# haoyu94/RoITr

Measured on AMD Instinct MI355X. Metric: point-cloud pairs/s, higher is better.
Workload: dtype f32; 1 GPU; 3DMatch-sized synthetic pairs: 5000 pts/cloud src+tgt, fp32, 3DMatch test settings (P=256 patches x 64 pts, 100 Sinkhorn iterations), full RIGA_v2 forward; n_points=5000, weights=closed-form, variant 'selective' (roitr_amd/weights.py); normals: field, cloud=uniform, correspondences_found=66241517

## Files before the change

### include/roitr_engine.h

```cpp
#ifndef ROITR_ENGINE_H
#define ROITR_ENGINE_H

#include <stddef.h>

#ifdef __cplusplus
extern "C" {
#endif

#ifndef ROITR_POINTOPS_H
typedef struct ihipStream_t* roitr_stream_t;
#endif

typedef struct RoitrGemm {
    int M, N, K;
    const float* A; const float* A2; int lda; const int* a_idx; int a_limit;
    const float* W; int ldw; const int* w_idx; int w_limit;
    const float* bias; float alpha; int relu;
    float* C; int ldc;
    int batch; long sA, sW, sC, sBias, sAidx, sWidx;
    const int* seg_off; int seg_a0, seg_w0;
    const float* ln_gamma; const float* ln_beta; const float* ln_res; const int* ln_res_idx; const float* ln_post;
    int ln_relu; float ln_eps;
    int bf16;
    const float* A_cat; int lda_cat; int k_cat;
// ... 24 lines not shown
                      roitr_stream_t stream);
int roitr_segment_mean(int b, int C, const float* x, const int* offset, float* out, roitr_stream_t stream);
int roitr_sinusoid(long rows, int C, const float* vals, const float* div_term, float* out, roitr_stream_t stream);
int roitr_geo_embed(long rows, int C, int angle_k, const float* d_idx, const float* a_idx, const float* div_term,
                    const float* Wd, const float* bd, const float* Wa, const float* ba, float* out, roitr_stream_t stream);
int roitr_split3_bf16(long n, const float* src, unsigned short* dst, roitr_stream_t stream);
int roitr_geo_embed_split(long rows, int C, int angle_k, const float* d_idx, const float* a_idx, const float* div_term,
                          const unsigned short* Wd3, const float* bd, const unsigned short* Wa3, const float* ba, float* out,
                          roitr_stream_t stream);
int roitr_geo_embed_bf16(long rows, int C, int angle_k, const float* d_idx, const float* a_idx, const float* div_term,
                         const unsigned short* Wd, const float* bd, const unsigned short* Wa, const float* ba, float* out,
                         roitr_stream_t stream);
int roitr_geo_embed_bf16_out(long rows, int C, int angle_k, const float* d_idx, const float* a_idx, const float* div_term,
                             const unsigned short* Wd, const float* bd, const unsigned short* Wa, const float* ba,
                             unsigned short* out, roitr_stream_t stream);
size_t roitr_geo_table_floats(int C, int n_int_d, int n_int_a);
int roitr_geo_table_build(int C, const float* div_term, const float* Wd, const float* bd, const float* Wa, const float* ba,
                          float interval, int n_int_d, int n_int_a, float* table, double* fit);
int roitr_geo_embed_table(long rows, int C, int angle_k, const float* d_idx, const float* a_idx, const float* table, float interval,
                          int n_int_d, int n_int_a, const float* div_term, const float* Wd, const float* bd, const float* Wa,
                          const float* ba, void* out, int out_bf16, roitr_stream_t stream);
int roitr_geo_combine(long rows, int C, int k, const float* pd, const float* pa, float* out, roitr_stream_t stream);
int roitr_gather_rows(long rows, int C, const float* in, const int* idx, int limit, float* out, roitr_stream_t stream);
int roitr_compose_idx(int n, const int* outer, const int* inner, int* out, roitr_stream_t stream);
int roitr_calc_ppf(int m, int k, const float* centre_xyz, const float* centre_normals, const float* ref_xyz,
                   const float* ref_normals, const int* group_idx, float* out, roitr_stream_t stream);

typedef struct RoitrLocalAttn {
    int M, K, H, heads;
    const float* q; int ldq;
    const float* k; int ldk;
    const float* v; int ldv;
    const int* group_idx; const float* ppf;
    const float* wvpe; const float* bvpe;
    float scale;
    float* out; int ldo;
    const void* node_order;
    int bf16;
    const float* wpe; const float* bpe;
} RoitrLocalAttn;
int roitr_local_attention(const RoitrLocalAttn* a, roitr_stream_t stream);
int roitr_build_pfold(int H, int heads, const float* wpe, const float* bpe, float* pfold, roitr_stream_t stream);

typedef struct RoitrLocalAttnFold {
    int M, in_dim, H;
    const float* x; int ldx;
// ... 59 lines not shown
int roitr_local_weights_reorder_host(const float* src, int rows, int k, int ldw, float* dst);

int roitr_geo_indices(int rows, const float* pts, const int* offset, const int* cloud_of_row, const long* eoff,
                      float sigma_d, float sigma_a, int angle_k, int n_max, float* d_idx, float* a_idx, roitr_stream_t stream);

typedef struct RoitrMha {
    int q_row0, q_rows, C, heads;
    const float* q; int ldq;
    const float* k; int ldk;
    const float* v; int ldv;
    const int* offset; const int* cloud_of_row; const int* partner;
    const float* E; const long* eoff; const float* qt; const float* bp;
    float scale; int nk_max;
    float* out; int ldo;
    float* ebar;
    int e_bf16;
} RoitrMha;
int roitr_mha(const RoitrMha* a, roitr_stream_t stream);


int roitr_point_to_node_partition(int b, int n_points, int n_nodes, const float* pts, const int* pt_offset,
                                  const float* nodes, const int* node_offset, const int* cloud_of_node, int limit,
                                  int* p2n, float* p2n_dist, int* node_masks, int* knn_idx, int* knn_mask, roitr_stream_t stream);

typedef struct RoitrCoarse {
    int pairs, C, num_corr, dual_norm, max_ref, max_src;
    const float* feats; const int* node_offset; const int* node_masks;
    float* scratch; long scratch_stride;
    int* tgt_corr; int* src_corr; float* corr_scores; int* n_corr;
    const float* xy; long xy_stride; int xy_ld;
    int lds_cap;
} RoitrCoarse;
size_t roitr_coarse_scratch_floats(int n_ref, int n_src);
int roitr_coarse_matching(const RoitrCoarse* a, roitr_stream_t stream);
int roitr_adaptive_matching(const RoitrCoarse* a, int min_num, float threshold, roitr_stream_t stream);

int roitr_patch_offsets(int pairs, const int* n_corr, int slots, int* pair_off, roitr_stream_t stream);

typedef struct RoitrPatch {
    int pairs, num_corr, limit;
    const int* n_corr; const int* tgt_corr; const int* src_corr;
    const int* node_offset; const int* pt_offset; const int* knn_idx; const int* knn_mask; const float* points;
    int* tgt_rows; int* src_rows; int* tgt_masks; int* src_masks; float* tgt_pts; float* src_pts;
    const int* pair_off; int slots;
} RoitrPatch;
int roitr_patch_gather(const RoitrPatch* a, roitr_stream_t stream);
// ... 73 lines not shown
    float* matching_scores;
    float* out_tgt_pts; float* out_src_pts; float* out_scores; int* out_patch;
    int* fine_offsets;
    int* n_out;
    float* gt_node_occ;
    int* gt_corr_idx;
    float* gt_corr_overlaps;
    int* gt_corr_count;
    void* inputs_ready;
    int* patch_offsets;
    int* pair_starts;
    int patch_slots;
} RoitrForwardIO;

void* roitr_engine_create(const RoitrEngineConfig* cfg);
void roitr_engine_destroy(void* engine);
int roitr_engine_set_param(void* engine, const char* name, const float* device_ptr, long numel);
int roitr_engine_finalize(void* engine, roitr_stream_t stream);
int roitr_engine_geo_table_info(void* engine, double* info);
int roitr_engine_forward(void* engine, const RoitrForwardIO* io, roitr_stream_t stream);
int roitr_engine_forward_graph(void* engine, const RoitrForwardIO* io, roitr_stream_t stream);
int roitr_engine_graph_count(void* engine);
int roitr_engine_set_phase_overlap(void* engine, int on);
int roitr_engine_scratch_info(void* engine, long* out5);
int roitr_engine_set_tap(void* engine, const char* name, void* device_ptr);
int roitr_engine_set_inject(void* engine, const char* name, const void* device_ptr);
void roitr_level_sizes(int n, int* out4);


int roitr_inlier_counts(int pairs, const int* starts, const float* src_pts, const float* tgt_pts, const float* rot,
                        const float* trans, float radius, int* inliers, roitr_stream_t stream);
int roitr_coarse_hits(int pairs, int num_corr, const int* n_corr, const int* tgt_corr, const int* src_corr, int gt_cap,
                      const int* gt_idx, const float* gt_overlaps, const int* gt_count, float acceptance_overlap, int* hits,
                      roitr_stream_t stream);


size_t roitr_registration_workspace_bytes(int pairs, int total_rows, int iterations, int chunks);
int roitr_ransac_correspondences(int pairs, const int* starts, int total_rows, const float* src_pts, const float* tgt_pts,
                                 const float* scores, const unsigned int* pair_keys, int sample_mode, int n_points, int ransac_n,
                                 float distance_threshold, float edge_similarity, int iterations, int refine_iters, int refine_weighted,
                                 unsigned long long seed, int chunks, void* workspace, size_t workspace_bytes, float* transforms,
                                 int* inliers, int* best_iteration, int* valid_hypotheses, int* n_used, int* selected,
                                 roitr_stream_t stream);
int roitr_ransac_samples(int pairs, const int* n, const unsigned int* pair_keys, unsigned long long seed, int it0, int count, int* out,
                         roitr_stream_t stream);
int roitr_weighted_procrustes(int batch, int n, const float* src_pts, const float* tgt_pts, const float* weights, float weight_thresh,
// ... 57 lines not shown
```

### roitr_amd/csrc/engine.cpp

```cpp
#include <hip/hip_runtime.h>
#include <math.h>
#include <stdio.h>
#include <string.h>

#include <map>
#include <string>
#include <vector>

#include "common.h"
#include "prof.h"
#include "roitr_engine.h"
#include "roitr_pointops.h"

#define CHK(x)                    \
    do {                          \
        int s__ = (x);            \
        if (s__ != 0) return s__; \
    } while (0)

namespace {

constexpr int HEADS = 4;
constexpr int GRID_MIN_POINTS = 768;

// ... 87 lines not shown
    hipStream_t side = nullptr;
    enum Ev {
        EV_MAIN_BEGIN,
        EV_LEVEL2_GEOM_DONE,
        EV_LEVEL3_GEOM_DONE,
        EV_LEVEL4_GEOM_DONE,
        EV_LEVEL1_WS_FREE,
        EV_EMBED_DONE,
        EV_NN3_DONE,
        EV_TAIL_DONE,
        EV_ERROR_JOIN,
        EV_DESC_COPIED,
        EV_LEVEL1_GROUPS_READY,
        EV_ENCODER_DONE,
        EV_BRANCH_DONE,
        EV_BRANCH_ERROR_JOIN,
        NEV
    };
    static Ev ev_level_done(int l) { return (Ev)(EV_LEVEL2_GEOM_DONE + l - 1); }
    hipEvent_t ev[NEV] = {};
    bool side_forked = false;
    hipStream_t branch = nullptr;
    int phase_overlap = 1;
    bool branch_forked = false;
    bool on_branch = false;
    std::string err;
    hipStream_t fin_stream = nullptr;
    struct GraphEntry {
        std::vector<long> key;
        hipGraph_t graph = nullptr; hipGraphExec_t exec = nullptr;
        char* pin = nullptr; size_t pin_cap = 0;
        long epoch = -1;
        bool warmed = false, failed = false;
        unsigned long stamp = 0;
    };
    std::vector<GraphEntry> graphs;
    long arena_epoch = 0;
    unsigned long graph_clock = 0;
    char* capture_pin = nullptr;
    std::map<std::pair<const float*, long>, unsigned short*> x3;
    std::vector<const float*> frag_weights;
};

thread_local Engine* g_engine = nullptr;

int use_x3(RoitrGemm& g, hipStream_t st)
// ... 782 lines not shown
                    break;
                }
            }
        }
    }
    if (E.warena.fail) { roitr_set_error("derived-weight arena exhausted", __FILE__, __LINE__); return ROITR_ERR_ARG; }
    E.finalized = true;
    return 0;
}

extern "C" int roitr_engine_geo_table_info(void* h, double* info)
{
    Engine& E = *(Engine*)h;
    if (!E.geo_tab) return 0;
    info[0] = E.geo_tab_h; info[1] = E.geo_tab_nd; info[2] = E.geo_tab_na;
    for (int q = 0; q < 6; ++q) info[3 + q] = E.geo_tab_fit[q];
    return 1;
}

static constexpr float GRID_OCC = 6.0f;

static constexpr int BRANCH_MIN_NODES = 8192;

static constexpr int AHEAD_MAX_PAIRS = 128;

static int forward_body(Engine& E, const RoitrForwardIO* io, hipStream_t st);

static int forward_joined(Engine& E, const RoitrForwardIO* io, hipStream_t st)
{
    E.side_forked = false; E.branch_forked = false; E.cur_par = -1; E.garena_short = false;
    const int rc = forward_body(E, io, st);
    if (rc != ROITR_OK && E.branch_forked && E.branch && E.ev[Engine::EV_BRANCH_ERROR_JOIN]) {
        if (hipEventRecord(E.ev[Engine::EV_BRANCH_ERROR_JOIN], E.branch) == hipSuccess) (void)hipStreamWaitEvent(st, E.ev[Engine::EV_BRANCH_ERROR_JOIN], 0);
        else (void)hipStreamSynchronize(E.branch);
    }
    if (rc != ROITR_OK && E.side_forked && E.side && E.ev[Engine::EV_ERROR_JOIN]) {
        if (hipEventRecord(E.ev[Engine::EV_ERROR_JOIN], E.side) == hipSuccess) (void)hipStreamWaitEvent(st, E.ev[Engine::EV_ERROR_JOIN], 0);
        else (void)hipStreamSynchronize(E.side);
    }
    return rc;
}

extern "C" int roitr_engine_forward(void* h, const RoitrForwardIO* io, hipStream_t st)
{
    Engine& E = *(Engine*)h;
    g_engine = &E;
// ... 334 lines not shown
            CHK(roitr_geo_embed_bf16_out(etot, C4, 3, S.d_idx, S.a_idx, E.geo_div, E.proj_d.wb, E.proj_d.b, E.proj_a.wb, E.proj_a.b,
                                         reinterpret_cast<unsigned short*>(S.Emb), sd));
        else if (E.cfg.operand_dtype == 1 && E.proj_d.wb && E.proj_a.wb)
            CHK(roitr_geo_embed_bf16(etot, C4, 3, S.d_idx, S.a_idx, E.geo_div, E.proj_d.wb, E.proj_d.b, E.proj_a.wb, E.proj_a.b, S.Emb, sd));
        else
            CHK(roitr_geo_embed(etot, C4, 3, S.d_idx, S.a_idx, E.geo_div, E.proj_d.w, E.proj_d.b, E.proj_a.w, E.proj_a.b, S.Emb, sd));
    }
    ROITR_HIP(hipEventRecord(E.ev[Engine::EV_EMBED_DONE], sd));
    return ROITR_OK;
}

int issue_tail(Engine& E, const RoitrForwardIO* io, const Plan& P, const GeoBufs& S)
{
    const Levels& V = P.V; const Desc& D = S.D; hipStream_t sd = P.sd;
    const int B = P.B, NC = P.NC, T1 = P.T1, T4 = P.T4, LIM = P.LIM;
    for (int l = 2; l >= 0; --l)
        CHK(roitr_knnquery_ex(NC, V.T[l + 1], V.T[l], 3, S.p[l + 1], S.p[l], D.off[l + 1], D.off[l], S.i3[l], S.d3[l], nullptr, nullptr, nullptr,
                              nullptr, S.grid[l + 1] ? 1 : 0, V.T[l], S.knn_ws[l + 1], sd));
    ROITR_HIP(hipEventRecord(E.ev[Engine::EV_NN3_DONE], sd));
    if (P.full_ahead) ROITR_HIP(hipStreamWaitEvent(sd, E.ev[Engine::EV_MAIN_BEGIN], 0));
    CHK(roitr_compose_idx(V.T[2], S.down[1], S.down[2], S.c3, sd));
    CHK(roitr_compose_idx(T4, S.c3, S.down[3], S.c4, sd));
    CHK(roitr_gather_rows(T4, 3, S.pts_out, S.c4, 0, S.node_xyz, sd));
    CHK(roitr_point_to_node_partition(NC, T1, T4, S.pts_out, D.off[0], S.node_xyz, D.off[3], D.cloud_of_node, LIM, S.p2n, S.p2nd, S.node_masks,
                                      S.kidx, S.kmask, sd));
    if (P.gt) {
        const int Tsp = P.Tsp, Ttp = P.Ttp;
        CHK(roitr_build_padded_clouds(B, T1, S.pts_out, D.off[0], io->rot, io->trans, S.gt_pad, S.gt_poff, sd));
        const float* src_p = S.gt_pad; const float* tgt_p = S.gt_pad + (size_t)Tsp * 3;
        const int* off_s = S.gt_poff; const int* off_t = S.gt_poff + 2 * B;
        const int use_grid = (Tsp > GRID_MIN_POINTS * B) ? 1 : 0;
        if (io->gt_node_occ) {
            float* d2p = S.gt_d2p;
            if (use_grid) CHK(roitr_knn_build_grid(B, Tsp, Ttp, src_p, off_s, S.gt_ws_s, sd));
            const float occ_cap2 = E.cfg.occlusion_radius * E.cfg.occlusion_radius * 1.01f;
            CHK(roitr_knn_within(B, Tsp, Ttp, src_p, tgt_p, off_s, off_t, occ_cap2, d2p + Tsp, use_grid, Ttp, S.gt_ws_s, sd));
            if (use_grid) CHK(roitr_knn_build_grid(B, Ttp, Tsp, tgt_p, off_t, S.gt_ws_t, sd));
            CHK(roitr_knn_within(B, Ttp, Tsp, tgt_p, src_p, off_t, off_s, occ_cap2, d2p, use_grid, Tsp, S.gt_ws_t, sd));
            CHK(roitr_node_occlusion_score(T4, LIM, D.cloud_of_node, D.off[0], S.kidx, S.kmask, S.node_masks, d2p, E.cfg.occlusion_radius,
                                           io->gt_node_occ, sd));
        }
        if (P.gt_corr) {
            const long ms = (long)V.nmax[3] * V.nmax[3];
            RoitrNodeCorr nc; memset(&nc, 0, sizeof(nc));
            nc.pairs = B; nc.limit = LIM; nc.max_nodes = V.nmax[3]; nc.pos_radius = E.cfg.matching_radius;
            nc.nodes = S.node_xyz; nc.node_offset = D.off[3]; nc.node_masks = S.node_masks; nc.points = S.pts_out; nc.pt_offset = D.off[0];
            nc.knn_idx = S.kidx; nc.knn_mask = S.kmask; nc.rot = io->rot; nc.trans = io->trans; nc.overlap = S.gt_om; nc.mat_stride = ms;
            nc.out_idx = io->gt_corr_idx; nc.out_overlap = io->gt_corr_overlaps; nc.out_count = io->gt_corr_count;
// ... 17 lines not shown
    CHK(roitr_knnquery_ex(NC, V.T[0], V.T[0], E.nsample[0] + 1, S.p[0], S.p[0], D.off[0], D.off[0], nullptr, nullptr, S.g_self[0], S.ppf_self[0],
                          S.nrm[0], S.nrm[0], S.grid[0] ? 1 : 0, T1, S.knn_ws[0], s0));
    if (P.knn0_ahead) {
        ROITR_HIP(hipEventRecord(E.ev[Engine::EV_LEVEL1_GROUPS_READY], sd));
        ROITR_HIP(hipStreamWaitEvent(st, E.ev[Engine::EV_LEVEL1_GROUPS_READY], 0));
        ROITR_HIP(hipEventRecord(E.ev[Engine::EV_MAIN_BEGIN], st));
    } else
        ROITR_HIP(hipEventRecord(E.ev[Engine::EV_LEVEL1_WS_FREE], st));
    if (P.ahead) CHK(sample_level(P, S, 1));

    if (!P.full_ahead) ROITR_HIP(hipStreamWaitEvent(sd, E.ev[Engine::EV_MAIN_BEGIN], 0));
    E.side_forked = true;
    for (int l = 1; l < 4; ++l) {
        const int K = E.nsample[l];
        if (!(P.ahead && l == 1)) CHK(sample_level(P, S, l));
        if (S.grid[l]) {
            CHK(roitr_knn_build_grid_ex(NC, V.T[l], V.T[l - 1], S.p[l], D.off[l], S.knn_ws[l], GRID_OCC, sd));
            S.order[l] = roitr_knn_sorted_points(NC, V.T[l], V.T[l - 1], S.knn_ws[l]);
        }
        CHK(roitr_knnquery_ex(NC, V.T[l], V.T[l], K + 1, S.p[l], S.p[l], D.off[l], D.off[l], nullptr, nullptr, S.g_self[l], S.ppf_self[l], S.nrm[l],
                              S.nrm[l], S.grid[l] ? 1 : 0, V.T[l - 1], S.knn_ws[l], sd));
        if (l == 1 && !P.knn0_ahead) ROITR_HIP(hipStreamWaitEvent(sd, E.ev[Engine::EV_LEVEL1_WS_FREE], 0));
        const int mcap_prev = l - 1 == 0 ? T1 : V.T[l - 2];
        CHK(roitr_knnquery_ex(NC, V.T[l - 1], V.T[l], K + 1, S.p[l - 1], S.p[l], D.off[l - 1], D.off[l], nullptr, nullptr, S.g_td[l],
                              S.ppf_td[l], S.nrm[l - 1], S.nrm[l], S.grid[l - 1] ? 1 : 0, mcap_prev, S.knn_ws[l - 1], sd));
        ROITR_HIP(hipEventRecord(E.ev[Engine::ev_level_done(l)], sd));
    }
    CHK(issue_embedding(E, P, S));
    return issue_tail(E, io, P, S);
}

int encoder(Engine& E, const RoitrForwardIO* io, const Plan& P, const GeoBufs& S, Feats& F)
{
    const Levels& V = P.V; const int T1 = P.T1; hipStream_t st = P.st; Arena& A = E.arena;
    const float* xin = io->feats;
    for (int l = 0; l < 4; ++l) {
        const int K = E.nsample[l], pl = E.planes[l];
        if (l > 0) {
            ROITR_HIP(hipStreamWaitEvent(st, E.ev[Engine::ev_level_done(l)], 0));
            CHK(tap(E, st, "fps." + std::to_string(l + 1), S.down[l], sizeof(int) * V.T[l]));
        }
        CHK(tap(E, st, "group.self." + std::to_string(l + 1), S.g_self[l], sizeof(int) * (size_t)V.T[l] * K));
        CHK(tap(E, st, "ppf.self." + std::to_string(l + 1), S.ppf_self[l], sizeof(float) * (size_t)V.T[l] * K * 4));
        if (l > 0) {
            CHK(tap(E, st, "group.td." + std::to_string(l + 1), S.g_td[l], sizeof(int) * (size_t)V.T[l] * K));
            CHK(tap(E, st, "ppf.td." + std::to_string(l + 1), S.ppf_td[l], sizeof(float) * (size_t)V.T[l] * K * 4));
        }
        float* a = A.get<float>((size_t)V.T[l] * pl);
// ... 281 lines not shown
    if (!forked) CHK(coarse_front(E, P, S, F, R));
    CHK(heads_and_matching(E, io, P, F, R));
    roitr_prof_end(ROITR_PROF_PH_MATCH, st);
    roitr_prof_end(ROITR_PROF_PH_FORWARD, st);
    return 0;
}

extern "C" int roitr_engine_scratch_info(void* h, long* out5)
{
    Engine& E = *(Engine*)h;
    out5[0] = (long)E.arena.cap; out5[1] = (long)E.arena.peak; out5[2] = (long)E.barena.cap; out5[3] = (long)E.barena.peak;
    out5[4] = E.on_branch ? 1 : 0;
    return ROITR_OK;
}

extern "C" int roitr_engine_set_phase_overlap(void* h, int on)
{
    Engine& E = *(Engine*)h;
    const int mode = on == 0 ? 0 : on == 2 ? 2 : 1;
    if (E.phase_overlap != mode) { E.phase_overlap = mode; E.arena_epoch++; }
    return ROITR_OK;
}


extern "C" int roitr_engine_forward_graph(void* h, const RoitrForwardIO* io, hipStream_t st)
{
    Engine& E = *(Engine*)h;
    if (!E.finalized) { roitr_set_error("engine not finalized", __FILE__, __LINE__); return ROITR_ERR_ARG; }
    if (!st || roitr_prof_is_enabled() || !E.taps.empty() || !E.injects.empty() || io->pairs <= 0) return roitr_engine_forward(h, io, st);
    std::vector<long> key;
    key.push_back(io->pairs);
    long t4 = 0;
    for (int c = 0; c < 2 * io->pairs; ++c) { key.push_back(io->n_points[c]); int s4[4]; roitr_level_sizes(io->n_points[c], s4); t4 += s4[3]; }
    {
        const void* const* pp = reinterpret_cast<const void* const*>(&io->points_geom);
        const size_t n_ptr = (reinterpret_cast<const char*>(&io->patch_slots) - reinterpret_cast<const char*>(&io->points_geom)) / sizeof(void*);
        for (size_t i = 0; i < n_ptr; ++i) key.push_back((long)(uintptr_t)pp[i]);
        key.push_back(io->patch_slots);
    }
    Engine::GraphEntry* ge = nullptr;
    for (auto& g : E.graphs) if (g.key == key) { ge = &g; break; }
    if (!ge) {
        if (E.graphs.size() >= 16) {
            size_t lru = 0;
            for (size_t i = 1; i < E.graphs.size(); ++i) if (E.graphs[i].stamp < E.graphs[lru].stamp) lru = i;
            auto& g = E.graphs[lru];
// ... 57 lines not shown
```

### roitr_amd/csrc/matching.hip

```cpp
#include "common.h"
#include <cstdio>
#include <cstdlib>
#include <type_traits>
#include "prof.h"
#include "roitr_engine.h"

namespace {

__device__ __forceinline__ float sq_norm3(float x, float y, float z)
{
#pragma clang fp contract(off)
    const float a = x * x, b = y * y, c = z * z;
    return (a + b) + c;
}
__device__ __forceinline__ float square_distance3(float sx, float sy, float sz, float s2, float tx, float ty, float tz, float t2)
{
#pragma clang fp contract(off)
    const float m = sx * tx;
    const float xy = __fmaf_rn(sz, tz, __fmaf_rn(sy, ty, m));
    const float a = -2.0f * xy;
    const float b = a + s2;
    return fmaxf(b + t2, 1e-12f);
}

__global__ __launch_bounds__(256) void p2n_assign_kernel(int n_points, const float* __restrict__ pts, const int* __restrict__ pt_offset,
                                                         const float* __restrict__ nodes, const int* __restrict__ node_offset, int b,
                                                         int* __restrict__ p2n, float* __restrict__ p2n_dist, int* __restrict__ node_masks)
{
    const int i = blockIdx.x * 256 + threadIdx.x;
    if (i >= n_points) return;
    const int c = segment_of(i, pt_offset, b);
    const int ns = c == 0 ? 0 : node_offset[c - 1], ne = node_offset[c];
    const float px = pts[(size_t)i * 3], py = pts[(size_t)i * 3 + 1], pz = pts[(size_t)i * 3 + 2];
    const float p2 = sq_norm3(px, py, pz);
    float best = INFINITY; int bi = ns;
    for (int j = ns; j < ne; ++j) {
        const float nx = nodes[(size_t)j * 3], ny = nodes[(size_t)j * 3 + 1], nz = nodes[(size_t)j * 3 + 2];
        const float d = square_distance3(nx, ny, nz, sq_norm3(nx, ny, nz), px, py, pz, p2);
        if (d < best) { best = d; bi = j; }
    }
    p2n[i] = bi - ns;
    p2n_dist[i] = best;
    node_masks[bi] = 1;
}

template <int THREADS>
__device__ __forceinline__ void block_bitonic_sort(unsigned long long* keys, int cap, int tid)
{
    for (int k = 2; k <= cap; k <<= 1) {
        for (int j = k >> 1; j > 0; j >>= 1) {
            for (int e = tid; e < cap; e += THREADS) {
                const int p = e ^ j;
                if (p > e) {
                    const unsigned long long x = keys[e], y = keys[p];
                    const bool up = (e & k) == 0;
                    if ((x > y) == up) { keys[e] = y; keys[p] = x; }
                }
            }
            __syncthreads();
        }
    }
}

constexpr int P2N_CAP = 2048;
__global__ __launch_bounds__(256) void p2n_topk_kernel(const int* __restrict__ pt_offset, const int* __restrict__ node_offset,
                                                       const int* __restrict__ cloud_of_node, const int* __restrict__ p2n,
                                                       const float* __restrict__ p2n_dist, int limit, int* __restrict__ knn_idx,
                                                       int* __restrict__ knn_mask)
{
    __shared__ unsigned long long keys[P2N_CAP];
    __shared__ unsigned long long red[4];
    __shared__ unsigned long long last_s;
    __shared__ int cnt_s;
    const int node = blockIdx.x;
    const int c = cloud_of_node[node];
    const int ps = c == 0 ? 0 : pt_offset[c - 1], pe = pt_offset[c];
    const int local = node - (c == 0 ? 0 : node_offset[c - 1]);
    const int tid = threadIdx.x, lane = tid & 63, wave = tid >> 6;
    if (tid == 0) cnt_s = 0;
    __syncthreads();
    for (int j = ps + tid; j < pe; j += 256) {
        if (p2n[j] == local) {
            const int pos = atomicAdd(&cnt_s, 1);
            if (pos < P2N_CAP) keys[pos] = ((unsigned long long)__float_as_uint(p2n_dist[j]) << 32) | (unsigned)(j - ps);
        }
    }
    __syncthreads();
    const int count = cnt_s;
    if (count <= P2N_CAP) {
        int cap = 64;
        while (cap < count) cap <<= 1;
        for (int e = count + tid; e < cap; e += 256) keys[e] = ~0ull;
        __syncthreads();
        block_bitonic_sort<256>(keys, cap, tid);
        for (int t = tid; t < limit; t += 256) {
            const bool ok = t < count;
            knn_idx[(size_t)node * limit + t] = ok ? (int)(unsigned)keys[t] : (pe - ps);
            knn_mask[(size_t)node * limit + t] = ok ? 1 : 0;
        }
        return;
// ... 640 lines not shown
    if (a.global_scores) {
        const PatchSlot ps = patch_slot(patch, a.pairs, a.num_corr, a.n_corr, a.pair_off);
        g = a.global_scores[(size_t)ps.pair * a.num_corr + ps.p];
    }
    const long cap = a.out_cap > 0 ? a.out_cap : 0x7fffffffL;
#pragma unroll
    for (int u = 0; u < per; ++u) {
        const int e = tid * per + u;
        if (((fw[u >> 2] >> (8 * (u & 3))) & 1u) && pos < cap) {
            const int i = e / L, j = e % L;
            const float* rp = a.row_pts + ((size_t)patch * L + i) * 3;
            const float* cp = a.col_pts + ((size_t)patch * L + j) * 3;
            a.out_row_pts[(size_t)pos * 3] = rp[0]; a.out_row_pts[(size_t)pos * 3 + 1] = rp[1]; a.out_row_pts[(size_t)pos * 3 + 2] = rp[2];
            a.out_col_pts[(size_t)pos * 3] = cp[0]; a.out_col_pts[(size_t)pos * 3 + 1] = cp[1]; a.out_col_pts[(size_t)pos * 3 + 2] = cp[2];
            a.out_scores[pos] = expf(sc[i * (L + 1) + j]) * g;
            if (a.out_patch) a.out_patch[pos] = patch;
            ++pos;
        }
    }
}

}

extern "C" int roitr_point_to_node_partition(int b, int n_points, int n_nodes, const float* pts, const int* pt_offset,
                                             const float* nodes, const int* node_offset, const int* cloud_of_node, int limit,
                                             int* p2n, float* p2n_dist, int* node_masks, int* knn_idx, int* knn_mask, hipStream_t stream)
{
    if (n_points <= 0 || n_nodes <= 0) return ROITR_OK;
    ROITR_HIP(hipMemsetAsync(node_masks, 0, sizeof(int) * (size_t)n_nodes, stream));
    p2n_assign_kernel<<<div_up(n_points, 256), 256, 0, stream>>>(n_points, pts, pt_offset, nodes, node_offset, b, p2n, p2n_dist, node_masks);
    ROITR_LAUNCH_CHECK();
    p2n_topk_kernel<<<n_nodes, 256, 0, stream>>>(pt_offset, node_offset, cloud_of_node, p2n, p2n_dist, limit, knn_idx, knn_mask);
    ROITR_LAUNCH_CHECK();
    return ROITR_OK;
}

extern "C" size_t roitr_coarse_scratch_floats(int n_ref, int n_src)
{
    const size_t total = (size_t)n_ref * n_src;
    const size_t spill_keys = total > COARSE_LDS_KEYS ? ((total + COARSE_LDS_KEYS - 1) / COARSE_LDS_KEYS) * 1024 + 64 : 0;
    return total + n_ref + n_src + 16 + 2 * spill_keys;
}

extern "C" int roitr_coarse_matching(const RoitrCoarse* a, hipStream_t stream)
{
    if (a->pairs <= 0) return ROITR_OK;
    long cap = 1;
    while (cap < (long)a->max_ref * a->max_src) cap <<= 1;
    if (cap > COARSE_LDS_KEYS) cap = COARSE_LDS_KEYS;
    if (a->num_corr > 1024) return ROITR_ERR_UNSUPPORTED;
    ROITR_GRANT_LDS(coarse_match_kernel, 128 * 1024);
    RoitrCoarse c = *a;
    c.lds_cap = (int)cap;
    coarse_match_kernel<<<a->pairs, 1024, cap * 8, stream>>>(c);
    ROITR_LAUNCH_CHECK();
    return ROITR_OK;
}
// ... 152 lines not shown
```

### roitr_amd/csrc/nn_ops.hip

```cpp
#include "common.h"
#include "roitr_engine.h"

namespace {

template <int VPL>
__global__ __launch_bounds__(256) void add_layernorm_kernel(int M, int C, const float* __restrict__ x, const float* __restrict__ res,
                                                            const int* __restrict__ res_idx, const float* __restrict__ gamma,
                                                            const float* __restrict__ beta, const float* __restrict__ post, int relu,
                                                            float eps, float* __restrict__ out, const float* __restrict__ ip_feat = nullptr,
                                                            const int* __restrict__ ip_idx = nullptr, const float* __restrict__ ip_dist2 = nullptr)
{
    const int lane = threadIdx.x & 63;
    const int row = blockIdx.x * 4 + (threadIdx.x >> 6);
    if (row >= M) return;
    const float* xr = x + (size_t)row * C;
    const float* rr = nullptr;
    if (res) rr = res + (size_t)(res_idx ? res_idx[row] : row) * C;
    float v[VPL];
    float s = 0.f;
#pragma unroll
    for (int i = 0; i < VPL; ++i) {
        const int c = lane + 64 * i;
        float t = 0.f;
        if (c < C) { t = xr[c]; if (rr) t += rr[c]; }
// ... 126 lines not shown
}

__global__ void geo_combine_kernel(long total, int C, int k, const float* __restrict__ pd, const float* __restrict__ pa, float* __restrict__ out)
{
    for (long t = blockIdx.x * 256L + threadIdx.x; t < total; t += gridDim.x * 256L) {
        const long r = t / C;
        const int c = (int)(t % C);
        float m = pa[(r * k) * C + c];
        for (int j = 1; j < k; ++j) m = fmaxf(m, pa[(r * k + j) * C + c]);
        out[t] = pd[t] + m;
    }
}

__global__ void gather_rows_kernel(long total, int C, const float* __restrict__ in, const int* __restrict__ idx, int limit, float* __restrict__ out)
{
    for (long t = blockIdx.x * 256L + threadIdx.x; t < total; t += gridDim.x * 256L) {
        const long r = t / C;
        const int c = (int)(t % C);
        const int s = idx[r];
        out[t] = (s >= 0 && (limit <= 0 || s < limit)) ? in[(size_t)s * C + c] : 0.f;
    }
}

__global__ void compose_idx_kernel(int n, const int* __restrict__ outer, const int* __restrict__ inner, int* __restrict__ out)
{
    const int t = blockIdx.x * 256 + threadIdx.x;
    if (t < n) out[t] = outer[inner[t]];
}

inline int ew_blocks(long total) { long b = (total + 255) / 256; return (int)(b > 8192 ? 8192 : (b < 1 ? 1 : b)); }

}

extern "C" int roitr_add_layernorm(int M, int C, const float* x, const float* res, const int* res_idx, const float* gamma,
                                   const float* beta, const float* post_add, int relu, float eps, float* out, hipStream_t stream)
{
    if (M <= 0) return ROITR_OK;
    if (C > 1024) return ROITR_ERR_UNSUPPORTED;
    const int blocks = div_up(M, 4);
#define LN_CASE(V) add_layernorm_kernel<V><<<blocks, 256, 0, stream>>>(M, C, x, res, res_idx, gamma, beta, post_add, relu, eps, out)
    if (C <= 64) LN_CASE(1); else if (C <= 128) LN_CASE(2); else if (C <= 256) LN_CASE(4); else if (C <= 512) LN_CASE(8); else LN_CASE(16);
#undef LN_CASE
    ROITR_LAUNCH_CHECK();
    return ROITR_OK;
}

// ... 71 lines not shown
    sinusoid_kernel<<<ew_blocks(total), 256, 0, stream>>>(total, C / 2, vals, div_term, (float2*)out);
    ROITR_LAUNCH_CHECK();
    return ROITR_OK;
}

extern "C" int roitr_geo_combine(long rows, int C, int k, const float* pd, const float* pa, float* out, hipStream_t stream)
{
    const long total = rows * C;
    if (total <= 0) return ROITR_OK;
    geo_combine_kernel<<<ew_blocks(total), 256, 0, stream>>>(total, C, k, pd, pa, out);
    ROITR_LAUNCH_CHECK();
    return ROITR_OK;
}

extern "C" int roitr_gather_rows(long rows, int C, const float* in, const int* idx, int limit, float* out, hipStream_t stream)
{
    const long total = rows * C;
    if (total <= 0) return ROITR_OK;
    gather_rows_kernel<<<ew_blocks(total), 256, 0, stream>>>(total, C, in, idx, limit, out);
    ROITR_LAUNCH_CHECK();
    return ROITR_OK;
}

extern "C" int roitr_compose_idx(int n, const int* outer, const int* inner, int* out, hipStream_t stream)
{
    if (n <= 0) return ROITR_OK;
    compose_idx_kernel<<<div_up(n, 256), 256, 0, stream>>>(n, outer, inner, out);
    ROITR_LAUNCH_CHECK();
    return ROITR_OK;
}
```

### roitr_amd/ops.py

```python
import torch

from . import _lib as L


def _i32c(t):
    return t.to(torch.int32).contiguous()


def calc_ppf(points, point_normals, ref_points, ref_normals, group_idx):
    m, k = group_idx.shape
    out = torch.empty((m, k, 4), dtype=torch.float32, device=points.device)
    grp = _i32c(group_idx)
    L.check(L.lib().roitr_calc_ppf(m, k, L.ptr(points.contiguous()), L.ptr(point_normals.contiguous()),
                                   L.ptr(ref_points.contiguous()), L.ptr(ref_normals.contiguous()), L.ptr(grp), L.ptr(out),
                                   L.stream_ptr()), "calc_ppf")
    return out


def calc_ppf_gpu(points, point_normals, patches, patch_normals):
    m, k, _ = patches.shape
    grp = torch.arange(m * k, dtype=torch.int32, device=points.device).view(m, k)
    return calc_ppf(points, point_normals, patches.reshape(-1, 3), patch_normals.reshape(-1, 3), grp)


# ... 391 lines not shown

def segment_mean(x, offset):
    x, off = _c(x), _c(offset, torch.int32)
    b, C = int(off.shape[0]), int(x.shape[1])
    out = torch.empty((b, C), dtype=torch.float32, device=x.device)
    L.check(L.lib().roitr_segment_mean(b, C, L.ptr(x), L.ptr(off), L.ptr(out), L.stream_ptr()), "segment_mean")
    return out


def interp3_add(feat, idx, dist2, base=None):
    feat, idx, dist2, base = _c(feat), _c(idx, torch.int32), _c(dist2), _c(base)
    n, C = int(idx.shape[0]), int(feat.shape[1])
    out = torch.empty((n, C), dtype=torch.float32, device=feat.device)
    L.check(L.lib().roitr_interp3_add(n, C, L.ptr(feat), L.ptr(idx), L.ptr(dist2), L.ptr(base), L.ptr(out), L.stream_ptr()), "interp3_add")
    return out


def gather_rows(x, idx, limit=0):
    x, idx = _c(x), _c(idx, torch.int32)
    rows, C = int(idx.shape[0]), int(x.shape[1])
    out = torch.empty((rows, C), dtype=torch.float32, device=x.device)
    L.check(L.lib().roitr_gather_rows(rows, C, L.ptr(x), L.ptr(idx), int(limit), L.ptr(out), L.stream_ptr()), "gather_rows")
    return out


def compose_idx(outer, inner):
    outer, inner = _c(outer, torch.int32), _c(inner, torch.int32)
    out = torch.empty_like(inner)
    L.check(L.lib().roitr_compose_idx(int(inner.shape[0]), L.ptr(outer), L.ptr(inner), L.ptr(out), L.stream_ptr()), "compose_idx")
    return out


def transpose(x, out=None):
    rows, cols = int(x.shape[0]), int(x.shape[1])
    if out is None:
        out = torch.empty((cols, rows), dtype=torch.float32, device=x.device)
    for t, shape in ((x, (rows, cols)), (out, (cols, rows))):
        if t.dtype != torch.float32 or tuple(t.shape) != shape or t.stride(1) != 1 or t.stride(0) < shape[1]:
            raise L.RoitrError("transpose: float32 (rows, cols) -> (cols, rows) with contiguous rows")
    L.check(L.lib().roitr_transpose(rows, cols, L.ptr(x), int(x.stride(0)), L.ptr(out), int(out.stride(0)), L.stream_ptr()), "transpose")
    return out


def add_vectors(a, b):
    a, b = _c(a), _c(b)
    if a.shape != b.shape:
# ... 253 lines not shown
```

### roitr_amd/riga.py

```python
import ctypes
import math
import time

import numpy as np
import torch
import torch.nn as nn

from . import _args as A
from . import _lib as L


def _linear(prefix, out, inp):
    return [(prefix + ".weight", (out, inp), "param"), (prefix + ".bias", (out,), "param")]


def _norm(prefix, c):
    return [(prefix + ".weight", (c,), "param"), (prefix + ".bias", (c,), "param")]


def _local_transformer(prefix, inp, hidden, out):
    ent = [(prefix + ".embedding.embedding.div_term", (hidden // 2,), "buffer")]
    ent += _linear(prefix + ".embedding.proj", hidden, 4)
    ent += _linear(prefix + ".in_proj", hidden, inp)
    for n in ("proj_q", "proj_k", "proj_v", "proj_p", "proj_vp"):
# ... 210 lines not shown

    def _weights_signature(self):
        return [(t.data_ptr(), t._version) for m in self._holders for d in (m._parameters, m._buffers) for t in d.values() if t is not None]

    def _ensure_engine(self):
        if self._engine is None or (not self.weights_frozen and self._weights_signature() != self._engine_sig):
            self.sync_engine()

    def set_tap(self, name, tensor):
        self._ensure_engine()
        self._taps = getattr(self, "_taps", {})
        self._taps[name] = tensor
        L.lib().roitr_engine_set_tap(self._engine, name.encode(), L.ptr(tensor))

    def set_inject(self, name, tensor):
        self._ensure_engine()
        self._injects = getattr(self, "_injects", {})
        self._injects[name] = tensor
        L.lib().roitr_engine_set_inject(self._engine, name.encode(), L.ptr(tensor))

    def set_phase_overlap(self, on=1):
        self._ensure_engine()
        L.check(L.lib().roitr_engine_set_phase_overlap(self._engine, ctypes.c_int(int(on))), "set_phase_overlap")

    def scratch_info(self):
        self._ensure_engine()
        out = (ctypes.c_long * 5)()
        L.check(L.lib().roitr_engine_scratch_info(self._engine, out), "scratch_info")
        return {"main_cap": out[0], "main_peak": out[1], "branch_cap": out[2], "branch_fill": out[3], "on_branch_stream": bool(out[4])}

    PROF_CLASSES = {"fps_kernel": 0, "knn_query_kernel": 1, "grid_build_kernel": 2, "knn_replay_kernel": 3, "phase.geometry": 4,
                    "phase.encoder": 5, "phase.global_transformer": 6, "phase.decoder": 7, "phase.matching": 8,
                    "phase.forward": 9, "ot_kernel": 10, "local_attn_kernel": 11, "gemm_kernel.mfma_roofed": 12, "mha_kernel": 13,
                    "geo_embed_kernel": 14, "geo_table_kernel": 15, "geo_embed_reference_flops": 16, "local_block_kernel": 17,
                    "gemm_kernel.hbm_roofed": 18}

    @staticmethod
    def profile_reset(enable=True):
        lib = L.lib()
        lib.roitr_prof_enable(1 if enable else 0)
        lib.roitr_prof_reset()

    @classmethod
    def profile_read(cls, kernels_only=True):
        lib = L.lib()
        out = {}
# ... 305 lines not shown
```

Before: 6501 pairs/s.

## Fuse point-to-node partition per cloud and reuse self-kNN groups for top-down

Adds a single-kernel point-to-node partition that handles one cloud per block in shared memory (assign, count, bucket, rank), replacing the assign and top-k kernel pair when the clouds fit. Separately, the top-down neighbour groups at each level are now gathered from the previous level's self-kNN groups and PPF via the downsample index, instead of running a new kNN query, when K matches. Both aim to cut kernel launches and redundant search work. The top-down reuse assumes the self-kNN of the sampled points equals the queried neighbourhood, which only holds because the query points are a subset of the source cloud.

After: 6530 pairs/s (median of 2 runs). No clear change (+0.4%).

```diff
diff --git a/include/roitr_engine.h b/include/roitr_engine.h
--- a/include/roitr_engine.h
+++ b/include/roitr_engine.h
@@ -70,6 +70,8 @@
                           const float* ba, void* out, int out_bf16, roitr_stream_t stream);
 int roitr_geo_combine(long rows, int C, int k, const float* pd, const float* pa, float* out, roitr_stream_t stream);
 int roitr_gather_rows(long rows, int C, const float* in, const int* idx, int limit, float* out, roitr_stream_t stream);
+int roitr_gather_groups(long rows, int K, const int* g_in, const float* ppf_in, const int* idx, int* g_out, float* ppf_out,
+                        roitr_stream_t stream);
 int roitr_compose_idx(int n, const int* outer, const int* inner, int* out, roitr_stream_t stream);
 int roitr_calc_ppf(int m, int k, const float* centre_xyz, const float* centre_normals, const float* ref_xyz,
                    const float* ref_normals, const int* group_idx, float* out, roitr_stream_t stream);
@@ -175,6 +177,11 @@
 int roitr_point_to_node_partition(int b, int n_points, int n_nodes, const float* pts, const int* pt_offset,
                                   const float* nodes, const int* node_offset, const int* cloud_of_node, int limit,
                                   int* p2n, float* p2n_dist, int* node_masks, int* knn_idx, int* knn_mask, roitr_stream_t stream);
+int roitr_partition_cloud_limits(int* max_points, int* max_nodes);
+int roitr_point_to_node_partition_ex(int b, int n_points, int n_nodes, const float* pts, const int* pt_offset,
+                                     const float* nodes, const int* node_offset, const int* cloud_of_node, int limit,
+                                     int* p2n, float* p2n_dist, int* node_masks, int* knn_idx, int* knn_mask, int one_pass, int max_points,
+                                     int max_nodes, roitr_stream_t stream);
 
 typedef struct RoitrCoarse {
     int pairs, C, num_corr, dual_norm, max_ref, max_src;
@@ -294,6 +301,7 @@
 int roitr_engine_forward_graph(void* engine, const RoitrForwardIO* io, roitr_stream_t stream);
 int roitr_engine_graph_count(void* engine);
 int roitr_engine_set_phase_overlap(void* engine, int on);
+int roitr_engine_set_td_reuse(void* engine, int on);
 int roitr_engine_scratch_info(void* engine, long* out5);
 int roitr_engine_set_tap(void* engine, const char* name, void* device_ptr);
 int roitr_engine_set_inject(void* engine, const char* name, const void* device_ptr);
diff --git a/roitr_amd/csrc/engine.cpp b/roitr_amd/csrc/engine.cpp
--- a/roitr_amd/csrc/engine.cpp
+++ b/roitr_amd/csrc/engine.cpp
@@ -133,6 +133,7 @@
     bool side_forked = false;
     hipStream_t branch = nullptr;
     int phase_overlap = 1;
+    int td_reuse = 1;
     bool branch_forked = false;
     bool on_branch = false;
     std::string err;
@@ -961,6 +962,8 @@
 
 static constexpr int BRANCH_MIN_NODES = 8192;
 
+static constexpr int P2N_ONE_PASS_MIN_CLOUDS = 256;
+
 static constexpr int AHEAD_MAX_PAIRS = 128;
 
 static int forward_body(Engine& E, const RoitrForwardIO* io, hipStream_t st);
@@ -1341,8 +1344,8 @@
     CHK(roitr_compose_idx(V.T[2], S.down[1], S.down[2], S.c3, sd));
     CHK(roitr_compose_idx(T4, S.c3, S.down[3], S.c4, sd));
     CHK(roitr_gather_rows(T4, 3, S.pts_out, S.c4, 0, S.node_xyz, sd));
-    CHK(roitr_point_to_node_partition(NC, T1, T4, S.pts_out, D.off[0], S.node_xyz, D.off[3], D.cloud_of_node, LIM, S.p2n, S.p2nd, S.node_masks,
-                                      S.kidx, S.kmask, sd));
+    CHK(roitr_point_to_node_partition_ex(NC, T1, T4, S.pts_out, D.off[0], S.node_xyz, D.off[3], D.cloud_of_node, LIM, S.p2n, S.p2nd, S.node_masks,
+                                         S.kidx, S.kmask, NC >= P2N_ONE_PASS_MIN_CLOUDS ? 1 : 0, V.nmax[0], V.nmax[3], sd));
     if (P.gt) {
         const int Tsp = P.Tsp, Ttp = P.Ttp;
         CHK(roitr_build_padded_clouds(B, T1, S.pts_out, D.off[0], io->rot, io->trans, S.gt_pad, S.gt_poff, sd));
@@ -1406,8 +1409,11 @@
                               S.nrm[l], S.grid[l] ? 1 : 0, V.T[l - 1], S.knn_ws[l], sd));
         if (l == 1 && !P.knn0_ahead) ROITR_HIP(hipStreamWaitEvent(sd, E.ev[Engine::EV_LEVEL1_WS_FREE], 0));
         const int mcap_prev = l - 1 == 0 ? T1 : V.T[l - 2];
-        CHK(roitr_knnquery_ex(NC, V.T[l - 1], V.T[l], K + 1, S.p[l - 1], S.p[l], D.off[l - 1], D.off[l], nullptr, nullptr, S.g_td[l],
-                              S.ppf_td[l], S.nrm[l - 1], S.nrm[l], S.grid[l - 1] ? 1 : 0, mcap_prev, S.knn_ws[l - 1], sd));
+        if (E.td_reuse && K == E.nsample[l - 1])
+            CHK(roitr_gather_groups(V.T[l], K, S.g_self[l - 1], S.ppf_self[l - 1], S.down[l], S.g_td[l], S.ppf_td[l], sd));
+        else
+            CHK(roitr_knnquery_ex(NC, V.T[l - 1], V.T[l], K + 1, S.p[l - 1], S.p[l], D.off[l - 1], D.off[l], nullptr, nullptr, S.g_td[l],
+                                  S.ppf_td[l], S.nrm[l - 1], S.nrm[l], S.grid[l - 1] ? 1 : 0, mcap_prev, S.knn_ws[l - 1], sd));
         ROITR_HIP(hipEventRecord(E.ev[Engine::ev_level_done(l)], sd));
     }
     CHK(issue_embedding(E, P, S));
@@ -1735,6 +1741,14 @@
     return ROITR_OK;
 }
 
+extern "C" int roitr_engine_set_td_reuse(void* h, int on)
+{
+    Engine& E = *(Engine*)h;
+    const int mode = on ? 1 : 0;
+    if (E.td_reuse != mode) { E.td_reuse = mode; E.arena_epoch++; }
+    return ROITR_OK;
+}
+
 
 extern "C" int roitr_engine_forward_graph(void* h, const RoitrForwardIO* io, hipStream_t st)
 {
diff --git a/roitr_amd/csrc/matching.hip b/roitr_amd/csrc/matching.hip
--- a/roitr_amd/csrc/matching.hip
+++ b/roitr_amd/csrc/matching.hip
@@ -23,14 +23,115 @@
     return fmaxf(b + t2, 1e-12f);
 }
 
+constexpr int P2N_CLOUD_PTS = 6144;
+constexpr int P2N_CLOUD_NODES = 256;
+constexpr int P2N_CLOUD_PER = P2N_CLOUD_PTS / 256;
+static_assert(P2N_CLOUD_PER % 4 == 0 && P2N_CLOUD_PER * 256 == P2N_CLOUD_PTS, "four points per pass");
+__device__ __forceinline__ bool p2n_cloud_fits(int n_pts, int n_nodes) { return n_pts <= P2N_CLOUD_PTS && n_nodes >= 1 && n_nodes <= P2N_CLOUD_NODES; }
+
+__global__ __launch_bounds__(256) void p2n_cloud_kernel(const float* __restrict__ pts, const int* __restrict__ pt_offset,
+                                                        const float* __restrict__ nodes, const int* __restrict__ node_offset, int limit,
+                                                        int* __restrict__ p2n, float* __restrict__ p2n_dist, int* __restrict__ node_masks,
+                                                        int* __restrict__ knn_idx, int* __restrict__ knn_mask)
+{
+    static_assert(P2N_CLOUD_NODES <= 256, "one thread per node");
+    __shared__ unsigned long long keys[P2N_CLOUD_PTS];
+    __shared__ float4 nd[P2N_CLOUD_NODES];
+    __shared__ int cnt[P2N_CLOUD_NODES], cur[P2N_CLOUD_NODES], start[P2N_CLOUD_NODES + 1];
+    const int c = blockIdx.x, tid = threadIdx.x;
+    const int ps = c == 0 ? 0 : pt_offset[c - 1], np = pt_offset[c] - ps;
+    const int ns = c == 0 ? 0 : node_offset[c - 1], nn = node_offset[c] - ns;
+    if (!p2n_cloud_fits(np, nn)) return;
+    if (tid < nn) {
+        const float nx = nodes[(size_t)(ns + tid) * 3], ny = nodes[(size_t)(ns + tid) * 3 + 1], nz = nodes[(size_t)(ns + tid) * 3 + 2];
+        nd[tid] = make_float4(nx, ny, nz, sq_norm3(nx, ny, nz));
+        cnt[tid] = 0;
+    }
+    __syncthreads();
+    float dist_r[P2N_CLOUD_PER]; int own_r[P2N_CLOUD_PER];
+#pragma unroll
+    for (int t0 = 0; t0 < P2N_CLOUD_PER; t0 += 4) {
+        if (t0 * 256 >= np) break;
+        float px[4], py[4], pz[4], p2[4], best[4]; int bi[4];
+#pragma unroll
+        for (int u = 0; u < 4; ++u) {
+            const int i = (t0 + u) * 256 + tid;
+            const size_t g = (size_t)(ps + (i < np ? i : np - 1));
+            px[u] = pts[g * 3]; py[u] = pts[g * 3 + 1]; pz[u] = pts[g * 3 + 2];
+            p2[u] = sq_norm3(px[u], py[u], pz[u]);
+            best[u] = INFINITY; bi[u] = 0;
+        }
+        for (int j = 0; j < nn; ++j) {
+            const float4 n = nd[j];
+#pragma unroll
+            for (int u = 0; u < 4; ++u) {
+                const float d = square_distance3(n.x, n.y, n.z, n.w, px[u], py[u], pz[u], p2[u]);
+                if (d < best[u]) { best[u] = d; bi[u] = j; }
+            }
+        }
+#pragma unroll
+        for (int u = 0; u < 4; ++u) {
+            const int i = (t0 + u) * 256 + tid;
+            dist_r[t0 + u] = best[u]; own_r[t0 + u] = bi[u];
+            if (i < np) {
+                p2n[ps + i] = bi[u];
+                p2n_dist[ps + i] = best[u];
+                atomicAdd(&cnt[bi[u]], 1);
+            }
+        }
+    }
+    __syncthreads();
+    if (tid < nn) {
+        int s = 0;
+        for (int j = 0; j < tid; ++j) s += cnt[j];
+        start[tid] = s; cur[tid] = s;
+        if (tid == nn - 1) start[nn] = s + cnt[tid];
+        if (cnt[tid] > 0) node_masks[ns + tid] = 1;
+    }
+    __syncthreads();
+#pragma unroll
+    for (int t = 0; t < P2N_CLOUD_PER; ++t) {
+        const int i = t * 256 + tid;
+        if (i < np) {
+            const int pos = atomicAdd(&cur[own_r[t]], 1);
+            keys[pos] = ((unsigned long long)__float_as_uint(dist_r[t]) << 32) | (unsigned)i;
+        }
+    }
+    __syncthreads();
+    for (int e = tid; e < np; e += 256) {
+        int lo = 0, hi = nn;
+        while (hi - lo > 1) { const int mid = (lo + hi) >> 1; if (start[mid] <= e) lo = mid; else hi = mid; }
+        const unsigned long long key = keys[e];
+        const int s0 = start[lo], s1 = start[lo + 1];
+        int rank = 0, q = s0;
+        for (; q + 4 <= s1; q += 4) {
+            const unsigned long long k0 = keys[q], k1 = keys[q + 1], k2 = keys[q + 2], k3 = keys[q + 3];
+            rank += (k0 < key ? 1 : 0) + (k1 < key ? 1 : 0) + (k2 < key ? 1 : 0) + (k3 < key ? 1 : 0);
+        }
+        for (; q < s1; ++q) rank += keys[q] < key ? 1 : 0;
+        if (rank < limit) {
+            knn_idx[(size_t)(ns + lo) * limit + rank] = (int)(unsigned)key;
+            knn_mask[(size_t)(ns + lo) * limit + rank] = 1;
+        }
+    }
+    for (int q = tid; q < nn * limit; q += 256) {
+        const int node = q / limit, t = q - node * limit;
+        if (t >= cnt[node]) {
+            knn_idx[(size_t)(ns + node) * limit + t] = np;
+            knn_mask[(size_t)(ns + node) * limit + t] = 0;
+        }
+    }
+}
+
 __global__ __launch_bounds__(256) void p2n_assign_kernel(int n_points, const float* __restrict__ pts, const int* __restrict__ pt_offset,
-                                                         const float* __restrict__ nodes, const int* __restrict__ node_offset, int b,
+                                                         const float* __restrict__ nodes, const int* __restrict__ node_offset, int b, int one_pass,
                                                          int* __restrict__ p2n, float* __restrict__ p2n_dist, int* __restrict__ node_masks)
 {
     const int i = blockIdx.x * 256 + threadIdx.x;
     if (i >= n_points) return;
     const int c = segment_of(i, pt_offset, b);
     const int ns = c == 0 ? 0 : node_offset[c - 1], ne = node_offset[c];
+    if (one_pass && p2n_cloud_fits(pt_offset[c] - (c == 0 ? 0 : pt_offset[c - 1]), ne - ns)) return;
     const float px = pts[(size_t)i * 3], py = pts[(size_t)i * 3 + 1], pz = pts[(size_t)i * 3 + 2];
     const float p2 = sq_norm3(px, py, pz);
     float best = INFINITY; int bi = ns;
@@ -65,8 +166,8 @@
 constexpr int P2N_CAP = 2048;
 __global__ __launch_bounds__(256) void p2n_topk_kernel(const int* __restrict__ pt_offset, const int* __restrict__ node_offset,
                                                        const int* __restrict__ cloud_of_node, const int* __restrict__ p2n,
-                                                       const float* __restrict__ p2n_dist, int limit, int* __restrict__ knn_idx,
-                                                       int* __restrict__ knn_mask)
+                                                       const float* __restrict__ p2n_dist, int limit, int one_pass,
+                                                       int* __restrict__ knn_idx, int* __restrict__ knn_mask)
 {
     __shared__ unsigned long long keys[P2N_CAP];
     __shared__ unsigned long long red[4];
@@ -76,6 +177,7 @@
     const int c = cloud_of_node[node];
     const int ps = c == 0 ? 0 : pt_offset[c - 1], pe = pt_offset[c];
     const int local = node - (c == 0 ? 0 : node_offset[c - 1]);
+    if (one_pass && p2n_cloud_fits(pe - ps, node_offset[c] - (c == 0 ? 0 : node_offset[c - 1]))) return;
     const int tid = threadIdx.x, lane = tid & 63, wave = tid >> 6;
     if (tid == 0) cnt_s = 0;
     __syncthreads();
@@ -762,17 +864,38 @@
 
 }
 
+extern "C" int roitr_partition_cloud_limits(int* max_points, int* max_nodes)
+{
+    if (max_points) *max_points = P2N_CLOUD_PTS;
+    if (max_nodes) *max_nodes = P2N_CLOUD_NODES;
+    return ROITR_OK;
+}
+
+extern "C" int roitr_point_to_node_partition_ex(int b, int n_points, int n_nodes, const float* pts, const int* pt_offset,
+                                                const float* nodes, const int* node_offset, const int* cloud_of_node, int limit,
+                                                int* p2n, float* p2n_dist, int* node_masks, int* knn_idx, int* knn_mask, int one_pass,
+                                                int max_points, int max_nodes, hipStream_t stream)
+{
+    if (n_points <= 0 || n_nodes <= 0 || b <= 0) return ROITR_OK;
+    ROITR_HIP(hipMemsetAsync(node_masks, 0, sizeof(int) * (size_t)n_nodes, stream));
+    if (one_pass) {
+        p2n_cloud_kernel<<<b, 256, 0, stream>>>(pts, pt_offset, nodes, node_offset, limit, p2n, p2n_dist, node_masks, knn_idx, knn_mask);
+        ROITR_LAUNCH_CHECK();
+        if (max_points > 0 && max_nodes > 0 && max_points <= P2N_CLOUD_PTS && max_nodes <= P2N_CLOUD_NODES) return ROITR_OK;
+    }
+    p2n_assign_kernel<<<div_up(n_points, 256), 256, 0, stream>>>(n_points, pts, pt_offset, nodes, node_offset, b, one_pass, p2n, p2n_dist, node_masks);
+    ROITR_LAUNCH_CHECK();
+    p2n_topk_kernel<<<n_nodes, 256, 0, stream>>>(pt_offset, node_offset, cloud_of_node, p2n, p2n_dist, limit, one_pass, knn_idx, knn_mask);
+    ROITR_LAUNCH_CHECK();
+    return ROITR_OK;
+}
+
 extern "C" int roitr_point_to_node_partition(int b, int n_points, int n_nodes, const float* pts, const int* pt_offset,
                                              const float* nodes, const int* node_offset, const int* cloud_of_node, int limit,
                                              int* p2n, float* p2n_dist, int* node_masks, int* knn_idx, int* knn_mask, hipStream_t stream)
 {
-    if (n_points <= 0 || n_nodes <= 0) return ROITR_OK;
-    ROITR_HIP(hipMemsetAsync(node_masks, 0, sizeof(int) * (size_t)n_nodes, stream));
-    p2n_assign_kernel<<<div_up(n_points, 256), 256, 0, stream>>>(n_points, pts, pt_offset, nodes, node_offset, b, p2n, p2n_dist, node_masks);
-    ROITR_LAUNCH_CHECK();
-    p2n_topk_kernel<<<n_nodes, 256, 0, stream>>>(pt_offset, node_offset, cloud_of_node, p2n, p2n_dist, limit, knn_idx, knn_mask);
-    ROITR_LAUNCH_CHECK();
-    return ROITR_OK;
+    return roitr_point_to_node_partition_ex(b, n_points, n_nodes, pts, pt_offset, nodes, node_offset, cloud_of_node, limit, p2n, p2n_dist,
+                                            node_masks, knn_idx, knn_mask, 1, 0, 0, stream);
 }
 
 extern "C" size_t roitr_coarse_scratch_floats(int n_ref, int n_src)
diff --git a/roitr_amd/csrc/nn_ops.hip b/roitr_amd/csrc/nn_ops.hip
--- a/roitr_amd/csrc/nn_ops.hip
+++ b/roitr_amd/csrc/nn_ops.hip
@@ -172,6 +172,18 @@
     }
 }
 
+__global__ void gather_groups_kernel(long total, int K, const int* __restrict__ g_in, const float4* __restrict__ ppf_in, const int* __restrict__ idx,
+                                     int* __restrict__ g_out, float4* __restrict__ ppf_out)
+{
+    for (long t = blockIdx.x * 256L + threadIdx.x; t < total; t += gridDim.x * 256L) {
+        const long r = t / K;
+        const int k = (int)(t % K);
+        const size_t s = (size_t)idx[r] * K + k;
+        g_out[t] = g_in[s];
+        ppf_out[t] = ppf_in[s];
+    }
+}
+
 __global__ void compose_idx_kernel(int n, const int* __restrict__ outer, const int* __restrict__ inner, int* __restrict__ out)
 {
     const int t = blockIdx.x * 256 + threadIdx.x;
@@ -289,6 +301,17 @@
     return ROITR_OK;
 }
 
+extern "C" int roitr_gather_groups(long rows, int K, const int* g_in, const float* ppf_in, const int* idx, int* g_out, float* ppf_out,
+                                   hipStream_t stream)
+{
+    const long total = rows * K;
+    if (total <= 0) return ROITR_OK;
+    if (((uintptr_t)ppf_in | (uintptr_t)ppf_out) & 15) { roitr_set_error("gather_groups: ppf rows must be 16-byte aligned", __FILE__, __LINE__); return ROITR_ERR_ARG; }
+    gather_groups_kernel<<<ew_blocks(total), 256, 0, stream>>>(total, K, g_in, (const float4*)ppf_in, idx, g_out, (float4*)ppf_out);
+    ROITR_LAUNCH_CHECK();
+    return ROITR_OK;
+}
+
 extern "C" int roitr_compose_idx(int n, const int* outer, const int* inner, int* out, hipStream_t stream)
 {
     if (n <= 0) return ROITR_OK;
diff --git a/roitr_amd/ops.py b/roitr_amd/ops.py
--- a/roitr_amd/ops.py
+++ b/roitr_amd/ops.py
@@ -437,6 +437,18 @@
     out = torch.empty((rows, C), dtype=torch.float32, device=x.device)
     L.check(L.lib().roitr_gather_rows(rows, C, L.ptr(x), L.ptr(idx), int(limit), L.ptr(out), L.stream_ptr()), "gather_rows")
     return out
+
+
+def gather_groups(group_idx, ppf, idx):
+    g, p, idx = _c(group_idx, torch.int32), _c(ppf), _c(idx, torch.int32)
+    rows, K = int(idx.shape[0]), int(g.shape[1])
+    if tuple(p.shape) != (int(g.shape[0]), K, 4):
+        raise L.RoitrError("gather_groups: ppf must be (R, K, 4) for group_idx (R, K)")
+    g_out = torch.empty((rows, K), dtype=torch.int32, device=g.device)
+    p_out = torch.empty((rows, K, 4), dtype=torch.float32, device=g.device)
+    L.check(L.lib().roitr_gather_groups(ctypes.c_long(rows), K, L.ptr(g), L.ptr(p), L.ptr(idx), L.ptr(g_out), L.ptr(p_out), L.stream_ptr()),
+            "gather_groups")
+    return g_out, p_out
 
 
 def compose_idx(outer, inner):
diff --git a/roitr_amd/riga.py b/roitr_amd/riga.py
--- a/roitr_amd/riga.py
+++ b/roitr_amd/riga.py
@@ -256,6 +256,10 @@
     def set_phase_overlap(self, on=1):
         self._ensure_engine()
         L.check(L.lib().roitr_engine_set_phase_overlap(self._engine, ctypes.c_int(int(on))), "set_phase_overlap")
+
+    def set_td_reuse(self, on=True):
+        self._ensure_engine()
+        L.check(L.lib().roitr_engine_set_td_reuse(self._engine, ctypes.c_int(int(bool(on)))), "set_td_reuse")
 
     def scratch_info(self):
         self._ensure_engine()
```
